# EMI-Group/evogp

Measured on AMD Instinct MI355X. Metric: tree_evals_per_s, higher is better.
Workload: dtype f32; 1 GPU; BASELINE north_star / configs[2] shape: SymbolicRegression synthetic 10-var, GLOBAL pop=1000000 x 1024 datapoints, max_tree_len=64, funcs + - * /, one tree_SR_fitness pass over every rank's shard per step; global_pop=1000000, pop_per_gpu=1000000, datapoints=1024, var_len=10, max_tree_len=64, ranks=1, device_prewarm_calls=40

## Files before the change

### evogp_amd/_lib.py

```python
from __future__ import annotations

import ctypes as C
import os

_HERE = os.path.dirname(os.path.abspath(__file__))
LIB_PATH = os.environ.get("EVOGP_HIP_LIB") or os.path.join(_HERE, "lib", "libevogp_hip.so")

ABI_VERSION = 9

_vp = C.c_void_p
_u = C.c_uint
_i = C.c_int
_f = C.c_float

PROTOTYPES = {
    "evogp_hip_generate": [_u, _u, _u, _u, _u, _f, _f, _vp, _vp, _vp, _vp, _vp, _vp, _vp, _u, _vp],
    "evogp_hip_mutate": [_i, _i, _vp, _vp, _vp, _vp, _vp, _vp, _vp, _vp, _vp, _vp, _vp],
    "evogp_hip_crossover": [_i, _i, _i, _vp, _vp, _vp, _vp, _vp, _vp, _vp, _vp, _vp, _vp, _vp],
    "evogp_hip_evaluate": [_u, _u, _u, _u, _vp, _vp, _vp, _vp, _vp, _vp],
    "evogp_hip_sr_fitness": [_u, _u, _u, _u, _u, _i, _vp, _vp, _vp, _vp, _vp, _vp, _u, _vp],
    "evogp_hip_generate_masked": [_u, _u, _u, _u, _u, _f, _f, _vp, _vp, _vp, _vp, _vp, _vp, _vp, _u, _vp, _u, _vp],
    "evogp_hip_breed_default": [_i, _i, _i, _i, _vp, _vp, _vp, _vp, _vp, _u, _vp, _vp, _vp, _vp, _vp, _vp, _vp, _vp],
    "evogp_hip_breed_default_rows": [_i, _i, _i, _i, _vp, _vp, _vp, _vp, _vp, _u, _vp, _vp, _vp, _vp, _vp, _vp, _vp, _i, _i, _vp],
    "evogp_hip_breed_default_table": [_i, _i, _i, _i, _i, _vp, _vp, _vp, _vp, _vp, _u, _vp, _vp, _vp, _vp, _vp, _vp, _vp, _i, _i, _vp],
# ... 37 lines not shown
    "evogp_hip_sr_semantic_hash_workspace_bytes": [_u, C.POINTER(C.c_ulonglong)],
    "evogp_hip_sr_semantic_hash": [_u, _u, _u, _u, _u, _vp, _vp, _vp, _vp, _vp, _vp, _vp],
    "evogp_hip_sr_semantic_classes_workspace_bytes": [_u, C.POINTER(C.c_ulonglong)],
    "evogp_hip_sr_semantic_classes": [_u, _u, _u, _u, _u, _vp, _vp, _vp, _vp, _vp, _vp, _vp, _vp],
    "evogp_hip_sr_linear_scaling": [_u, _u, _u, _u, _u, _vp, _vp, _vp, _vp, _vp, _vp, _vp, _vp],
    "evogp_hip_sr_weighted_loss": [_u, _u, _u, _u, _u, _vp, _vp, _vp, _vp, _vp, _vp, _u, _i, C.c_double, _vp, _vp],
    "evogp_hip_sr_weighted_gradient": [_u, _u, _u, _u, _u, _vp, _vp, _vp, _vp, _vp, _vp, _i, C.c_double, _vp, _vp, _vp],
    "evogp_hip_sr_weighted_normal_eq": [_u, _u, _u, _u, _u, _vp, _vp, _vp, _vp, _vp, _vp, _vp, _vp, _vp],
    "evogp_hip_sr_weighted_scaling": [_u, _u, _u, _u, _u, _vp, _vp, _vp, _vp, _vp, _vp, _u, _vp, _vp, _vp],
    "evogp_hip_sr_input_gradient": [_u, _u, _u, _u, _u, _vp, _vp, _vp, _vp, _u, _vp, _vp, _vp, _vp],
    "evogp_hip_sr_derivative_loss": [_u, _u, _u, _u, _u, _vp, _vp, _vp, _vp, _vp, _vp, _u, _vp, _vp, _vp, _vp, _vp, _vp],
    "evogp_hip_sr_gene_fitness": [_u, _u, _u, _u, _u, _vp, _vp, _vp, _vp, _vp, _vp, _vp, _vp, _vp],
    "evogp_hip_wrap_linear":[_u, _u, _u, _vp, _vp, _vp, _vp, _vp, _vp, _vp, _vp, _vp],
    "evogp_hip_tree_intervals": [_u, _u, _u, _vp, _vp, _vp, _vp, _vp, _vp, _vp, _vp, _vp],
    "evogp_hip_tree_derivative_intervals": [_u, _u, _u, _vp, _vp, _vp, _vp, _vp, _u, _vp, _vp, _vp, _vp, _vp, _vp, _vp, _vp],
    "evogp_hip_tree_dimensions": [_u, _u, _u, _u, _vp, _vp, _vp, _vp, _vp, _i, _vp, _vp, _vp, _vp],
    "evogp_hip_tree_structure": [_u, _u, _u, _vp, _vp, _vp, _vp, _vp, _vp, _vp, _vp, _i, _i, _vp, _vp, _vp, _vp, _vp, _vp, _vp],
}

DEBUG_PROTOTYPES = {
    "evogp_hip_timer_begin": [_vp],
    "evogp_hip_timer_end": [_vp, C.POINTER(C.c_float)],
    "evogp_hip_debug_set_stats": [_vp],
    "evogp_hip_debug_compile_batch": [_i],
    "evogp_hip_debug_long_compiler": [_i],
    "evogp_hip_debug_twins": [_i],
    "evogp_hip_debug_tc_fold": [_i],
    "evogp_hip_debug_tc_end": [_i],
    "evogp_hip_debug_tc_nanpeek": [_i],
    "evogp_hip_debug_tc_nanpeek_raised": [],
    "evogp_hip_debug_tc_batches": [_i, _i],
    "evogp_hip_debug_tc_table": [_i],
    "evogp_hip_debug_tc_dense": [_i],
    "evogp_hip_debug_tc_table_entry": [_i, _i, C.POINTER(C.c_uint)],
    "evogp_hip_debug_profile": [_i],
    "evogp_hip_debug_profile_read": [C.POINTER(C.c_float), C.POINTER(C.c_int)],
    "evogp_hip_debug_tc_histogram": [_u, _vp, _i, _vp],
    "evogp_hip_debug_tc_nhandlers": [],
    "evogp_hip_debug_tc_program": [_u, _vp, _i],
    "evogp_hip_debug_forget_function_classes": [],
    "evogp_hip_debug_structural_mutate_given": [_i, _i, _i, _i, _i, _vp, _vp, _vp, _vp, _vp, _vp, _vp, _vp],
    "evogp_hip_debug_insert_mutate_given": [_i, _i, _i, _vp, _vp, _vp, _vp, _vp, _vp, _vp, _vp, _vp, _vp, _vp],
    "evogp_hip_debug_point_mutate_given": [_i, _i, _i, _i, _i, _i, _i, _i, _i, _vp, _vp, _vp, _vp, _vp, _vp, _vp, _vp, _vp, _vp, _vp, _vp, _vp, _vp],
    "evogp_hip_debug_lexicase": [_vp, _i],
    "evogp_hip_debug_pareto_rank": [_i],
}


def _load() -> C.CDLL:
    if not os.path.exists(LIB_PATH):
        raise ImportError(
            f"{LIB_PATH} is missing: build the HIP engine first "
            "(python -c 'import __graft_entry__ as g; g.build()'  or  make -C evogp_amd/csrc). "
            "evogp_amd has no CPU fallback."
        )
    lib = C.CDLL(LIB_PATH)
    for name, argtypes in list(PROTOTYPES.items()) + list(DEBUG_PROTOTYPES.items()):
        fn = getattr(lib, name)
        fn.argtypes = argtypes
        fn.restype = _i
    lib.evogp_hip_evaluate_workspace_bytes.argtypes = [_u, _u]
    lib.evogp_hip_evaluate_workspace_bytes.restype = C.c_size_t
    lib.evogp_hip_select_workspace_bytes.argtypes = []
    lib.evogp_hip_select_workspace_bytes.restype = C.c_size_t
    lib.evogp_hip_program_buffer_bytes.argtypes = []
    lib.evogp_hip_program_buffer_bytes.restype = C.c_ulonglong
# ... 17 lines not shown
```

### evogp_amd/csrc/sr_tc.hip

```cpp
#include "interp.hpp"
#include "launch.hpp"
#include "sr_params.hpp"
#include "tc_interp_k8.inc"
#include "tc_interp_k4.inc"
#include "tc_interp_k1.inc"

#include <atomic>
#include <cstddef>
#include <mutex>
#include <cstdio>
#include <vector>

namespace evogp {

struct TcCompileParams {
    const float *value;
    const int16_t *type;
    const int16_t *size;
    uint2 *prog;
    float *fitness;
    unsigned *marks;
    unsigned *zero_next;
    int pop, gp_len, var_len;
    uint32_t unary_mask;
// ... 35 lines not shown
static std::atomic<int> g_fold{-1};
static std::atomic<int> g_lean_end{-1};
static std::atomic<int> g_nanpeek{-1};
static std::atomic<int> g_nanpeek_raised{0};
static std::atomic<int> g_tc_batch{0}, g_tc_dynshift{-1};
static std::atomic<int> g_compile_batch{-2};
static std::atomic<int> g_word_table{-1};
static int tc_nan_trees() {
    static const int env_fold = env_int("EVOGP_TC_FOLD", 2);
    const int fo = g_fold.load(std::memory_order_relaxed);
    return fo >= 0 ? fo : (env_fold < 0 || env_fold > 2 ? 2 : env_fold);
}
static bool tc_lean_end() {
    static const int env_end = env_int("EVOGP_TC_END", 1);
    const int le = g_lean_end.load(std::memory_order_relaxed);
    return (le >= 0 ? le : env_end) != 0;
}
static bool tc_nanpeek(long n, int num_cus) {
    static const int env_peek = env_int("EVOGP_TC_NANPEEK", 1);
    const int np = g_nanpeek.load(std::memory_order_relaxed);
    return np >= 0 ? np != 0 : (env_peek == 2 || (env_peek == 1 && n >= 900l * num_cus));
}
static bool tc_word_table() {
    static const int env_table = env_int("EVOGP_TC_TABLE", 1);
    const int wt = g_word_table.load(std::memory_order_relaxed);
    return (wt >= 0 ? wt : env_table) != 0;
}
static std::atomic<int> g_dense{-1};
static bool tc_dense() {
    static const int env_dense = env_int("EVOGP_TC_DENSE", 1);
    const int de = g_dense.load(std::memory_order_relaxed);
    return (de >= 0 ? de : env_dense) != 0;
}
static_assert(EVOGP_TC_H_LEAF_V == EVOGP_TC_H_LEAF_C + 1, "TcCompileParams::leaf_id: the variable's word is the constant's + 1, as PUSH_V is PUSH_C + 1");
static_assert(kSentinelHeavy == 0x7FC0FEEDu, "gen/gen_tc_asm.py SENTINEL_HEAVY");

__device__ inline float fold_bin4_fast(int op, float x, float y) {
    return op == 0 ? x + y : op == 1 ? x - y : op == 2 ? x * y : (y == 0.0f ? __builtin_nanf("") : x / y);
}

__device__ inline uint32_t tc_word0(int id, int slot, uint32_t pf_bytes, uint32_t aux = 0u) {
    return ((pf_bytes >> 10) << 24) | ((aux & 0xFFu) << 16) | (uint32_t)(((slot & 1) * EVOGP_TC_NHANDLERS + id) * EVOGP_TC_SLOT);
}

static_assert(EVOGP_TC_H_PUSH_V == EVOGP_TC_H_PUSH_C + 1 && EVOGP_TC_H_DIVIP_CS == EVOGP_TC_H_DIVIP_SS + 2 && EVOGP_TC_H_DIVR_CV == EVOGP_TC_H_DIVR_SV + 2 &&
              EVOGP_TC_H_PUSH_C_NP == EVOGP_TC_H_ADD_SS_NP + 24 && EVOGP_TC_H_DIVIP_SS_NP == EVOGP_TC_H_ADD_SS_NP + 26 &&
              EVOGP_TC_H_DIVR_SV_NP == EVOGP_TC_H_ADD_SS_NP + 29, "gen/gen_tc_asm.py NOPF_TWINS");
__device__ inline int no_prefetch_delta(bool arith3, bool push_c, bool in_place, bool by_recip) {
    return arith3 ? (int)EVOGP_TC_H_ADD_SS_NP : push_c ? (int)EVOGP_TC_H_PUSH_C_NP - (int)EVOGP_TC_H_PUSH_C
         : in_place ? (int)EVOGP_TC_H_DIVIP_SS_NP - (int)EVOGP_TC_H_DIVIP_SS : by_recip ? (int)EVOGP_TC_H_DIVR_SV_NP - (int)EVOGP_TC_H_DIVR_SV : 0;
}
__device__ inline bool next_word_has_variable(const TcCompileParams &, unsigned long long keptwave, bool kept, bool uses_var, bool is_root) {
    const unsigned long long U = __ballot(kept & uses_var);
    return __builtin_amdgcn_inverse_ballot_w64((((~keptwave) + (U << 1)) & keptwave) | __ballot(is_root));
}

__device__ inline void division_by_reciprocal(const TcCompileParams &p, int &id, uint32_t pf, uint32_t d1, uint32_t &aux) {
    const bool sv = id == 3 * 8 + 1, vv = id == 3 * 8 + 5, cv = id == 3 * 8 + 7;
    const bool ok = (p.recip != 0u) & (sv | vv | cv);
    const uint32_t voff = vv ? d1 << 4 : pf;
    aux = ok ? (voff + p.recip) >> 10 : aux;
    id = ok ? (int)EVOGP_TC_H_DIVR_SV + (int)vv + 2 * (int)cv : id;
}

constexpr int kUnaryInv = 10;
constexpr int kUnaryZero = 11;
// ... 1908 lines not shown
                zr = (bperm(z, rl4) & fnr) | zlr;
            }
            Mnan |= Mfn & Mop3 & B(zr != 0);
        }
    }
    const int nanincl = (int)__builtin_amdgcn_mbcnt_hi((uint32_t)(Mnan >> 32), __builtin_amdgcn_mbcnt_lo((uint32_t)Mnan, 0u)) + seli(L(Mnan), 1, 0);
    const int both = (int)((uint32_t)inclf << 15) | (nanincl << 8) | above;
    const int at_end = bperm(both, (end - 1) << 2), before = bperm(both, (lo - 1) << 2);
    const int base = seli(lo > 0, before >> 15, 0);
    const int slot = above - (at_end & 0xFF);
    const int totf = (at_end >> 15) - base;
    const int hf = seli(L(Mkept), totf - (inclf - base - deltaf), 0);
    const M Mpz = Min & B(((at_end >> 8) & 127) != seli(lo > 0, (before >> 8) & 127, 0));
    const M Mhigh = B(hf > p.depth);
    if ((Min & (~M4 | Msb | Mhigh)) != 0ull) return false;
    uint32_t ids = ent_ids;
    if (p.twins) {
        const M Uk = B((ent_bits & kTcEntUsesKept) != 0u);
        const M nxt = (((~keptwave) + (Uk << 1)) & keptwave) | Mroot;
        ids = selu(L(nxt), ids, ids >> 8);
    }
    const M Minpl = B(hf + (int)(ent_bits & kTcEntRoomMask) <= p.depth - p.div_reserve);
    const int id = (int)(selu(L(Minpl), ids >> 16, ids) & 0xFFu);
    if (L(Mkept & ~Mpz)) *(uint2 *)(rec0 + (roff + (uint32_t)slot * 8u)) = make_uint2(tc_word0(id, slot, pf, aux), d1);
    if (L(Mroot)) {
        uint32_t nan_tree = tc_word0(EVOGP_TC_H_NAN_TREE, 0, 0u);
        asm volatile("" : "+v"(nan_tree));
        const uint32_t lastw = selu(L(Mpz), nan_tree, tc_word0(p.end_id, slot + 1, p.ydelta));
        *(uint2 *)(rec0 + (roff + (uint32_t)seli(L(Mpz), 0, slot + 1) * 8u)) = make_uint2(lastw, 0u);
    }
    return true;
}

template <int B>
__global__ __launch_bounds__(256) void tc_compile_dense_kernel(TcCompileParams p) {
    typedef unsigned long long M;
    extern __shared__ uint2 tc_table_lds[];
    const int lane = threadIdx.x & 63;
    const uint32_t wave = threadIdx.x >> 6;
    const uint32_t tab = wave * (uint32_t)kTcCodes;
    {
        const int half = p.recip != 0u ? 1 : 0;
#pragma unroll
        for (int c = lane; c < kTcCodes; c += 64) {
            const uint32_t bits = kTcWordTable.bits[half][c];
            tc_table_lds[tab + (uint32_t)c] = make_uint2(kTcWordTable.ids[half][c] + ((bits & kTcEntLeaf) ? (uint32_t)p.leaf_id * 0x0101u : 0u), bits);
        }
        __builtin_amdgcn_wave_barrier();
    }
    if (p.zero_next && blockIdx.x == 0)
        for (int i = threadIdx.x; i < kCallScratchWords; i += blockDim.x) p.zero_next[i] = 0u;
    const uint32_t wave_id = uni((blockIdx.x * blockDim.x + threadIdx.x) >> 6);
    const uint32_t t0 = wave_id * (uint32_t)B;
    if (t0 >= (uint32_t)p.pop) return;
    const int nb = (int)min((uint32_t)B, (uint32_t)p.pop - t0);
    const int Lr = p.gp_len;
    uint8_t *const fnidx = (uint8_t *)(tc_table_lds + (blockDim.x >> 6) * (uint32_t)kTcCodes) + wave * (uint32_t)(B * 32);
    const size_t node0 = (size_t)t0 * (uint32_t)Lr;
    const float *const value0 = p.value + node0;
    const int16_t *const type0 = p.type + node0, *const size0 = p.size + node0;
    char *const rec0 = (char *)p.prog + (size_t)t0 * p.rec;
    int raw = 1, ty0 = T_CONST;
    float val0 = 0.0f;
    if (lane < nb) {
        const uint32_t at = (uint32_t)__mul24(lane, Lr);
        raw = (int)*(const int16_t *)((const char *)size0 + at * 2u); ty0 = (int)*(const int16_t *)((const char *)type0 + at * 2u);
        val0 = *(const float *)((const char *)value0 + at * 4u);
    }
    const int lens = lane < nb ? max(1, min(raw, Lr)) : 0;
    bool bad = __builtin_amdgcn_ballot_w64(lane < nb && (raw <= 0 || raw > Lr || (raw & 1) == 0 || (raw == 1 && ty0 != T_VAR && ty0 != T_CONST))) != 0ull;
    int nfs = 0;
    if (!bad) {
        constexpr int G = 8;
        auto load8 = [&](int (&ty)[G], int b0) {
#pragma unroll
            for (int k = 0; k < G; ++k) {
                const int len = __builtin_amdgcn_readlane(lens, (b0 + k) & 63);
                ty[k] = T_CONST;
                if (b0 + k < B && len > 1 && lane < len) ty[k] = (int)*(const int16_t *)((const char *)type0 + (uint32_t)(__mul24(b0 + k, Lr) + lane) * 2u);
            }
        };
        int cur[G], nxt[G];
        load8(cur, 0);
#pragma unroll
        for (int b0 = 0; b0 < B; b0 += G) {
            if (b0 + G < B) load8(nxt, b0 + G);
#pragma unroll
            for (int k = 0; k < G; ++k) {
                const int b = b0 + k;
                const int len = __builtin_amdgcn_readlane(lens, b);
                if (len > 1) {
                    const int ty = cur[k];
                    const M fn = __builtin_amdgcn_ballot_w64(ty == T_BFUNC);
                    const M leaf = __builtin_amdgcn_ballot_w64(ty == T_VAR) | __builtin_amdgcn_ballot_w64(ty == T_CONST);
                    const int cnt = __popcll(fn);
                    bad |= ~(fn | leaf) != 0ull || 2 * cnt + 1 != len;
                    const int rank = (int)__builtin_amdgcn_mbcnt_hi((uint32_t)(fn >> 32), __builtin_amdgcn_mbcnt_lo((uint32_t)fn, 0u));
                    if (ty == T_BFUNC && rank < 32) fnidx[b * 32 + rank] = (uint8_t)lane;
                    nfs = lane == b ? cnt : nfs;
                }
            }
#pragma unroll
            for (int k = 0; k < G; ++k) cur[k] = nxt[k];
        }
        wave_lds_sync();
    }
    bool ok = !bad;
    if (ok) {
        if (lens == 1) {
            const bool isv = ty0 == T_VAR;
            const int v = max(0, min((int)val0, p.var_len - 1));
            const uint32_t pay = isv ? (uint32_t)v * p.var_stride : f2bits(val0);
            const uint32_t id = tc_table_lds[tab + (uint32_t)(kTcCodeOther + kTcCodeRoot) + (isv ? 0u : 1u)].x & 0xFFu;
            const bool nan = !isv && p.nan_trees != 0 && (pay << 1) > 0xFF000000u;
            uint2 *const r = (uint2 *)(rec0 + (uint32_t)__mul24(lane, (int)p.rec));
            if (nan) r[0] = make_uint2(tc_word0(EVOGP_TC_H_NAN_TREE, 0, 0u), 0u);
            else {
                r[0] = make_uint2(tc_word0((int)id, 0, isv ? pay : 0u, 0u), isv ? 0u : pay);
                r[1] = make_uint2(tc_word0(p.end_id, 1, p.ydelta), 0u);
            }
        }
        int sval = nfs | (lane << 8);
#pragma unroll
        for (int r = 2; r < 5; ++r) {
            const M ones = __builtin_amdgcn_ballot_w64((sval & (1 << r)) != 0);
            const int below1 = (int)__builtin_amdgcn_mbcnt_hi((uint32_t)(ones >> 32), __builtin_amdgcn_mbcnt_lo((uint32_t)ones, 0u));
            const int to = (sval & (1 << r)) ? below1 : __popcll(ones) + lane - below1;
            sval = __builtin_amdgcn_ds_permute(to << 2, sval);
        }
        const int slen = sval & 127;
        M left = __builtin_amdgcn_ballot_w64(slen > 0);
        struct Pass { M inm; int tb, lo, nf, i, sz, tyl, szl, tyr, szr; uint32_t row; float val, vall, valr; };
        auto plan = [&](Pass &n) {
            int used = 0, about = 0;
            while (true) {
                const M cand = __builtin_amdgcn_ballot_w64(slen <= 64 - used) & left;
                if (cand == 0ull) break;
                const int j = __builtin_ctzll(cand);
                left &= ~(1ull << j);
                const int sv = __builtin_amdgcn_readlane(sval, j), l = sv & 127;
                about = (uint32_t)(lane - used) < (uint32_t)l ? (sv | (used << 16)) : about;
                used += l;
                if (used >= 64) break;
            }
            n.inm = used >= 64 ? ~0ull : (1ull << used) - 1ull;
            n.tb = (about >> 8) & 255; n.lo = about >> 16; n.nf = about & 127;
            n.row = (uint32_t)__mul24(n.tb, Lr);
            n.i = 0; n.val = (float)F_ADD; n.sz = 3; n.tyl = T_CONST; n.vall = 0.0f; n.szl = 1; n.tyr = T_CONST; n.valr = 0.0f; n.szr = 1;
            if (lane < used) {
                n.i = min((int)fnidx[n.tb * 32 + lane - n.lo], 2 * n.nf);
                const uint32_t at = n.row + (uint32_t)n.i, atl = n.row + (uint32_t)min(n.i + 1, 2 * n.nf);
                n.val = *(const float *)((const char *)value0 + at * 4u); n.sz = (int)*(const int16_t *)((const char *)size0 + at * 2u);
                n.tyl = (int)*(const int16_t *)((const char *)type0 + atl * 2u); n.vall = *(const float *)((const char *)value0 + atl * 4u);
                n.szl = (int)*(const int16_t *)((const char *)size0 + atl * 2u);
            }
        };
        auto right = [&](Pass &n) {
            if (__builtin_amdgcn_inverse_ballot_w64(n.inm)) {
                const uint32_t at = n.row + (uint32_t)dense_right_child(n.i, n.szl, n.nf);
                n.tyr = (int)*(const int16_t *)((const char *)type0 + at * 2u); n.valr = *(const float *)((const char *)value0 + at * 4u);
                n.szr = (int)*(const int16_t *)((const char *)size0 + at * 2u);
            }
        };
        Pass a = {}, b = {};
        bool have_a = left != 0ull, have_b = false;
        if (have_a) plan(a);
        have_b = left != 0ull;
        if (have_b) plan(b);
        if (have_a) right(a);
        while (have_a) {
            const Pass c = a;
            if (have_b) right(b);
            a = b; have_a = have_b;
            have_b = left != 0ull;
            if (have_b) plan(b);
            const uint32_t roff = (uint32_t)__mul24(c.tb, (int)p.rec);
            ok = compile_dense_arith(p, rec0, roff, c.inm, c.lo, c.nf, c.i, c.val, c.sz, c.tyl, c.vall, c.szl, c.tyr, c.valr, c.szr, lane, tab);
            if (!ok) break;
        }
    }
    if (!ok) tc_packed_batch<B>(p, wave_id, t0, nb, lane, tab);
}


__device__ __attribute__((always_inline)) inline int compile_long_arith(const TcCompileParams &p, char *rec0, int t, int len, char *lds, int lane,
                                                           int ty0, float val0, int sz0, int ty1, float val1, int sz1, int lds_len) {
    auto any = [](bool c) -> bool { return __builtin_amdgcn_ballot_w64(c) != 0ull; };
    auto seli = [](bool c, int x, int y) -> int { return c ? x : y; };
    auto selu = [](bool c, uint32_t x, uint32_t y) -> uint32_t { return c ? x : y; };
    const int L = lds_len;
    uint32_t *ks_s = (uint32_t *)lds;
    uint32_t *pay_s = ks_s + L;
    uint32_t *ek_s = pay_s + L;
    uint32_t *ep_s = ek_s + L;
    int32_t *offh_s = (int32_t *)(ep_s + L);
    int32_t *end_s = offh_s + L;
    int16_t *pre_s = (int16_t *)(end_s + L + 1);
    const size_t row = (size_t)t * p.gp_len;
    const int nch = (len + 63) >> 6;
    constexpr uint32_t kULo = 2u | (3u << 4) | (4u << 8) | (15u << 12) | (15u << 16) | (15u << 20) | (8u << 24) | (9u << 28);
    constexpr uint32_t kUHi = 7u | ((uint32_t)UG_INV << 4) | (15u << 8) | (0u << 12) | (1u << 16) | (5u << 20) | (6u << 24) | (15u << 28);
    for (int c = 0; c < nch; ++c) {
        const int i = c * 64 + lane;
        const bool in = i < len;
        int ty = T_CONST, sz = 1;
        float val = 0.0f;
        if (in) {
            if (c == 0) { ty = ty0; val = val0; sz = sz0; }
            else if (c == 1) { ty = ty1; val = val1; sz = sz1; }
            else { ty = (int)p.type[row + i]; val = p.value[row + i]; sz = (int)p.size[row + i]; }
        }
        const uint32_t f = (uint32_t)val;
        const bool isV = ty == T_VAR, isC = ty == T_CONST, isBf = ty == T_BFUNC, isUf = ty == T_UFUNC;
        const uint32_t fi = f - (uint32_t)F_SIN;
// ... 953 lines not shown
            for (long w = 0; w < sw && w < n; ++w) sample += (n - 1 - w) / nwaves + 1;
            *mark_sample = (int)sample;
        }
        const size_t clds = 4 * tc_general_lds_bytes(p.gp_len);
        if (clds > 64 * 1024 && !d.attr_set[15]) {
            (void)hipFuncSetAttribute((const void *)tc_compile_general_kernel<true>, hipFuncAttributeMaxDynamicSharedMemorySize, 160 * 1024 - 1024);
            (void)hipGetLastError();
            d.attr_set[15] = true;
        }
        static const int env_packed_env = env_int("EVOGP_TC_PACKED", -1);
        const int set_packed = g_compile_batch.load(std::memory_order_relaxed);
        const int env_packed = set_packed != -2 ? set_packed : env_packed_env;
        static const int env_generic = env_int("EVOGP_TC_PACK_GENERIC", 1);
        const bool packed_mo = p.out_len > 1 && env_packed != 0 && env_generic != 0;
        const bool packed = (p.out_len == 1 && env_packed != 0) || packed_mo;
        if (packed) {
            const bool un = c.nblocks != 1;
            constexpr unsigned kOwnHandlers = (1u << F_ADD) | (1u << F_SUB) | (1u << F_MUL) | (1u << F_DIV) | (1u << F_SIN) | (1u << F_COS) | (1u << F_TAN) |
                                              (1u << F_LOG) | (1u << F_LOOSE_LOG) | (1u << F_EXP) | (1u << F_INV) | (1u << F_NEG) | (1u << F_ABS) |
                                              (1u << F_SQRT) | (1u << F_LOOSE_SQRT);
            const bool may_generic = p.func_mask == 0u || (p.func_mask & ~kOwnHandlers) != 0u;
            const int mode = packed_mo ? 3 : (c.general && p.hint_general && env_generic != 0 && may_generic) ? 2 : (un || c.gp_len > 64) ? 1 : 0;
            int B = n >= 400000 ? 32 : n >= 200000 ? 16 : 8;
            if (env_packed > 0) B = env_packed >= 64 ? 64 : env_packed >= 32 ? 32 : env_packed >= 16 ? 16 : 8;
            if (mode >= 2) B = B >= 16 ? 32 : 8;
            static const int env_pwg = env_int("EVOGP_TC_PACKED_WG", 0);
            const int wgw = env_pwg == 64 ? 1 : env_pwg == 256 ? 4 : n >= 120000 ? 1 : 4;
            const long pblocks = ((long)n + wgw * B - 1) / (wgw * B);
            if (first) *mark_sample = (int)std::min<long>(n, (long)kMarkSampleBlocks * 4 * B);
            learn_packed = c.learn != 0 && mode != 3;
            nan_words = c.nan_trees >= 1 && mode != 3;
            const dim3 grid((unsigned)pblocks), wg(64 * wgw);
            const bool longrows = c.gp_len > 64;
#define EVOGP_LAUNCH_MODE(BB, MM) \
            do { if (longrows) hipLaunchKernelGGL((tc_compile_packed_kernel<BB, MM, true>), grid, wg, 0, strm, c); \
                 else hipLaunchKernelGGL((tc_compile_packed_kernel<BB, MM, false>), grid, wg, 0, strm, c); } while (0)
#define EVOGP_LAUNCH_PACKED(BB) \
            do { if (mode == 1) EVOGP_LAUNCH_MODE(BB, 1); \
                 else if (tc_word_table() && tc_dense()) hipLaunchKernelGGL((tc_compile_dense_kernel<BB>), grid, wg, (size_t)wgw * (kTcCodes * sizeof(uint2) + BB * 32), strm, c); \
                 else if (tc_word_table()) hipLaunchKernelGGL((tc_compile_packed_kernel<BB, 0, false, true>), grid, wg, (size_t)wgw * kTcCodes * sizeof(uint2), strm, c); \
                 else hipLaunchKernelGGL((tc_compile_packed_kernel<BB, 0, false>), grid, wg, 0, strm, c); } while (0)
            if (mode == 3) { if (B == 32) EVOGP_LAUNCH_MODE(32, 3); else EVOGP_LAUNCH_MODE(8, 3); }
            else if (mode == 2) { if (B == 32) EVOGP_LAUNCH_MODE(32, 2); else EVOGP_LAUNCH_MODE(8, 2); }
            else if (B == 64) EVOGP_LAUNCH_PACKED(64);
            else if (B == 32) EVOGP_LAUNCH_PACKED(32);
            else if (B == 16) EVOGP_LAUNCH_PACKED(16);
            else EVOGP_LAUNCH_PACKED(8);
#undef EVOGP_LAUNCH_PACKED
#undef EVOGP_LAUNCH_MODE
        }
        if (packed_mo) {
            hipError_t le = hipGetLastError();
            if (le != hipSuccess) return le;
            if (p.gp_len > 64) launch_marked_general(c, n, strm);
        } else if (p.out_len == 1) {
            if (!packed) hipLaunchKernelGGL(tc_compile_kernel, dim3((unsigned)cblocks), dim3(256), 0, strm, c);
            hipError_t le = hipGetLastError();
            if (le != hipSuccess) return le;
            static const bool dbg_marks = getenv("EVOGP_DEBUG_MARKS") != nullptr;
            if (dbg_marks) {
                std::vector<uint32_t> h((size_t)n);
                (void)hipStreamSynchronize(strm);
                (void)hipMemcpy(h.data(), c.fitness, (size_t)n * 4, hipMemcpyDeviceToHost);
                int shown = 0;
                for (int t = 0; t < n && shown < 4; ++t)
                    if (h[t] == kSentinelGeneral || h[t] == kSentinelHeavy) {
                        std::vector<int16_t> ty(c.gp_len), sz(c.gp_len);
                        std::vector<float> va(c.gp_len);
                        (void)hipMemcpy(ty.data(), c.type + (size_t)t * c.gp_len, c.gp_len * 2, hipMemcpyDeviceToHost);
                        (void)hipMemcpy(sz.data(), c.size + (size_t)t * c.gp_len, c.gp_len * 2, hipMemcpyDeviceToHost);
                        (void)hipMemcpy(va.data(), c.value + (size_t)t * c.gp_len, c.gp_len * 4, hipMemcpyDeviceToHost);
                        fprintf(stderr, "[evogp] tree %d left %s: len %d:", lo + t, h[t] == kSentinelGeneral ? "to the general compiler" : "marked heavy", (int)sz[0]);
// ... 360 lines not shown
            for (int i = 0; i < 32; ++i) {
                const unsigned h = (w[i].x & 0xFFFFu) / EVOGP_TC_SLOT;
                if (h >= 2u * EVOGP_TC_NHANDLERS) break;
                const unsigned id = h % EVOGP_TC_NHANDLERS;
                atomicAdd(h_s + h, 1u);
                if (id == EVOGP_TC_H_END || id == EVOGP_TC_H_END_MO || id == EVOGP_TC_H_END_CLS || id == EVOGP_TC_H_SKIP || id == EVOGP_TC_H_NAN_TREE ||
                    id == EVOGP_TC_H_END_LEAN || id == EVOGP_TC_H_LEAF_C || id == EVOGP_TC_H_LEAF_V) break;
                if (id == EVOGP_TC_H_NEXT) { r += w[i].y; more = true; break; }
            }
        }
    }
    __syncthreads();
    for (int i = threadIdx.x; i < 2 * EVOGP_TC_NHANDLERS; i += blockDim.x)
        if (h_s[i]) atomicAdd(hist + i, (unsigned long long)h_s[i]);
}

hipError_t tc_histogram(int pop, unsigned long long *hist, int hist_len, hipStream_t stream) {
    int dev = 0;
    (void)hipGetDevice(&dev);
    TcDevice &d = g_tc[dev & 63];
    std::lock_guard<std::mutex> lock(d.mu);
    if (!d.last_records || d.last_pop <= 0 || hist_len < 2 * EVOGP_TC_NHANDLERS) return hipErrorInvalidValue;
    if (pop > d.last_pop) pop = d.last_pop;
    hipError_t e = hipMemsetAsync(hist, 0, (size_t)hist_len * sizeof(unsigned long long), stream);
    if (e != hipSuccess) return e;
    hipLaunchKernelGGL(tc_histogram_kernel, dim3((unsigned)((pop + 255) / 256)), dim3(256), 0, stream, (const uint2 *)d.last_records, pop, d.last_rec, hist);
    return hipGetLastError();
}

hipError_t launch_threaded_code(const SrParams &p, hipStream_t stream, bool *handled, int *mark_sample, int *mark_chunks) {
    *handled = false;
    *mark_sample = 0;
    *mark_chunks = 1;
    if (p.results != nullptr) return hipSuccess;
    if (p.classify && p.out_len < 2) return hipSuccess;
    int k = p.D > 256 ? 8 : (p.D > 64 ? 4 : 1);
    static const int env_wide = env_int("EVOGP_TC_WIDE", 1);
    bool wide = false;
    if (p.out_len > 1 && p.out_len + 3 > EVOGP_TC_K8_DEPTH && k == 8) {
        if (env_wide && p.out_len + 3 <= EVOGP_TC_K8W_DEPTH && !p.stats) wide = true; else k = 4;
    }
    if (p.out_len > 1 && p.out_len + 3 > EVOGP_TC_K4_DEPTH && k == 4) return hipSuccess;
    if (p.out_len > 1 && p.out_len + 3 > EVOGP_TC_K1_DEPTH) return hipSuccess;
    static const int env_k = env_int("EVOGP_TC_K", 0);
    if (env_k == 1 || env_k == 4 || env_k == 8) k = env_k;
#ifndef EVOGP_FUSED_STATS
    if (p.stats) return run_tc<8, true>(p, stream, handled, mark_sample, mark_chunks);
#endif
    const int dm = sr_division_mode();
#ifdef EVOGP_FUSED_STATS
    static const int env_fused = env_int("EVOGP_TC_FUSED", 1);
#else
    static const int env_fused = env_int("EVOGP_TC_FUSED", -1);
#endif
    const bool fused_ok = k == 8 && p.out_len == 1 && !p.classify && p.gp_len <= 64 && p.marks && !p.prof_mid;
    auto fused = [&]() -> hipError_t {
        return dm == 1 ? run_fused<1>(p, stream, handled, mark_sample, mark_chunks)
             : dm == 2 ? run_fused<2>(p, stream, handled, mark_sample, mark_chunks)
                       : run_fused<0>(p, stream, handled, mark_sample, mark_chunks);
    };
    if (env_fused == 1 && fused_ok && !p.hint_general) {
        hipError_t fe = fused();
        if (fe != hipSuccess || *handled) return fe;
    }
#define EVOGP_RUN_TC(F) (wide && k == 8 ? run_tc<8, false, F, true>(p, stream, handled, mark_sample, mark_chunks) \
                        : k == 8 ? run_tc<8, false, F>(p, stream, handled, mark_sample, mark_chunks) \
// ... 23 lines not shown
}

extern "C" int evogp_hip_debug_tc_end(int mode) {
    if (mode < -1 || mode > 1) return EVOGP_E_BADARG;
    evogp::g_lean_end.store(mode, std::memory_order_relaxed);
    return EVOGP_OK;
}

extern "C" int evogp_hip_debug_tc_nanpeek(int mode) {
    if (mode < -1 || mode > 1) return EVOGP_E_BADARG;
    evogp::g_nanpeek.store(mode, std::memory_order_relaxed);
    return EVOGP_OK;
}

extern "C" int evogp_hip_debug_tc_batches(int batch, int dyn_shift) {
    if (batch < 0 || batch > 64 || dyn_shift < -1 || dyn_shift > 3) return EVOGP_E_BADARG;
    evogp::g_tc_batch.store(batch, std::memory_order_relaxed);
    evogp::g_tc_dynshift.store(dyn_shift, std::memory_order_relaxed);
    return EVOGP_OK;
}

extern "C" int evogp_hip_debug_tc_nanpeek_raised(void) { return evogp::g_nanpeek_raised.load(std::memory_order_relaxed); }

extern "C" int evogp_hip_debug_tc_table(int mode) {
    if (mode < -1 || mode > 1) return EVOGP_E_BADARG;
    evogp::g_word_table.store(mode, std::memory_order_relaxed);
    return EVOGP_OK;
}

extern "C" int evogp_hip_debug_tc_dense(int mode) {
    if (mode < -1 || mode > 1) return EVOGP_E_BADARG;
    evogp::g_dense.store(mode, std::memory_order_relaxed);
    return EVOGP_OK;
}

extern "C" int evogp_hip_debug_tc_table_entry(int recip, int code, unsigned *entry) {
    if (recip < 0 || recip > 1 || code < 0 || code >= evogp::kTcCodes || !entry) return EVOGP_E_BADARG;
    entry[0] = evogp::kTcWordTableHost.ids[recip][code];
    entry[1] = evogp::kTcWordTableHost.bits[recip][code];
    return EVOGP_OK;
}

extern "C" int evogp_hip_debug_long_compiler(int fast) {
    if (fast < -1 || fast > 1) return EVOGP_E_BADARG;
    evogp::g_long_fast.store(fast, std::memory_order_relaxed);
    return EVOGP_OK;
}

extern "C" int evogp_hip_debug_compile_batch(int trees) {
    if (trees < -1 || trees > 64) return EVOGP_E_BADARG;
    evogp::g_compile_batch.store(trees, std::memory_order_relaxed);
    return EVOGP_OK;
}

extern "C" int evogp_hip_set_program_buffer_limit(unsigned long long bytes) {
    evogp::g_prog_limit.store(bytes, std::memory_order_relaxed);
    return EVOGP_OK;
}

extern "C" int evogp_hip_set_allocator(evogp_alloc_fn alloc, evogp_free_fn free_fn) {
    if ((alloc == nullptr) != (free_fn == nullptr)) return EVOGP_E_BADARG;
    for (auto &d : evogp::g_tc) {
        std::lock_guard<std::mutex> lock(d.mu);
        if (d.prog || d.graph_prog || !d.retired.empty() || !d.rings.empty() || d.spare_ring) return EVOGP_E_BADARG;
    }
    if (evogp::grad_workspaces_held() || evogp::case_workspaces_held()) return EVOGP_E_BADARG;
// ... 87 lines not shown
```

### include/evogp_hip_debug.h

```cpp
#ifndef EVOGP_HIP_DEBUG_H
#define EVOGP_HIP_DEBUG_H
#include "evogp_hip.h"
#ifdef __cplusplus
extern "C" {
#endif

int evogp_hip_timer_begin(evogp_stream_t stream);
int evogp_hip_timer_end(evogp_stream_t stream, float *elapsed_ms);

int evogp_hip_debug_set_stats(unsigned long long *device_counters);

int evogp_hip_debug_profile(int enable);
int evogp_hip_debug_profile_read(float *stage_ms , int *calls);

int evogp_hip_debug_compile_batch(int trees);
int evogp_hip_debug_long_compiler(int fast);
int evogp_hip_debug_twins(int mode);
int evogp_hip_debug_tc_fold(int mode);
int evogp_hip_debug_tc_end(int mode);
int evogp_hip_debug_tc_nanpeek(int mode);
int evogp_hip_debug_tc_nanpeek_raised(void);
int evogp_hip_debug_tc_batches(int batch, int dyn_shift);
int evogp_hip_debug_tc_table(int mode);
int evogp_hip_debug_tc_dense(int mode);
int evogp_hip_debug_tc_table_entry(int recip, int code, unsigned *entry);

int evogp_hip_debug_tc_histogram(unsigned pop, unsigned long long *device_hist, int hist_len, evogp_stream_t stream);
int evogp_hip_debug_tc_nhandlers(void);
int evogp_hip_debug_tc_program(unsigned tree, unsigned *host_words, int max_words);

int evogp_hip_debug_forget_function_classes(void);

int evogp_hip_debug_structural_mutate_given(int pop_size, int gp_len, int mode, int inner_is_offset, int skip_rows, const int *given,
                                            const float *value, const int16_t *type, const int16_t *size, float *value_res,
                                            int16_t *type_res, int16_t *size_res, evogp_stream_t stream);
int evogp_hip_debug_insert_mutate_given(int pop_size, int gp_len, int skip_rows, const int *given, const float *value, const int16_t *type,
                                        const int16_t *size, const float *donor_value, const int16_t *donor_type, const int16_t *donor_size,
                                        float *value_res, int16_t *type_res, int16_t *size_res, evogp_stream_t stream);
int evogp_hip_debug_point_mutate_given(int pop_size, int gp_len, int mode, int modify_output, int fix_roulette, int skip_rows, int input_len,
                                       int output_len, int n_consts, const unsigned char *target, const float *u, const int *var_idx,
                                       const int *const_idx, const int *out_idx, const float *value, const int16_t *type, const int16_t *size,
                                       const float *roulette_ufuncs, const float *roulette_bfuncs, const float *roulette_tfuncs,
                                       const float *const_samples, float *value_res, evogp_stream_t stream);

int evogp_hip_debug_lexicase(unsigned long long *device_counters, int stop_after);

int evogp_hip_debug_pareto_rank(int stop_after);

#ifdef __cplusplus
}
#endif
#endif
```

Baseline: 1930 billion tree-evals/s.

## Restructure dense tree compiler node stage with packed per-node metadata in LDS

The dense compile kernel's node scan now has each lane read four nodes at once with 8-byte loads. It covers four trees per wave step, classifies nodes with packed 16-bit ops, ranks function nodes with a DPP prefix scan, and writes a per-node meta byte (size and type class) to LDS. The plan stage then reads child sizes and types from that LDS meta instead of reloading type and size from global memory, and drops the separate right-child prefetch pass. It also loads child values only for leaves. The dense path is now taken only when gp_len is a multiple of four and the type and size buffers are 8-byte aligned. A device counter of fallbacks to the packed compiler is added for debugging, at the cost of more LDS per wave.

```diff
diff --git a/evogp_amd/_lib.py b/evogp_amd/_lib.py
--- a/evogp_amd/_lib.py
+++ b/evogp_amd/_lib.py
@@ -93,6 +93,7 @@
     "evogp_hip_debug_tc_batches": [_i, _i],
     "evogp_hip_debug_tc_table": [_i],
     "evogp_hip_debug_tc_dense": [_i],
+    "evogp_hip_debug_tc_dense_fallbacks": [],
     "evogp_hip_debug_tc_table_entry": [_i, _i, C.POINTER(C.c_uint)],
     "evogp_hip_debug_profile": [_i],
     "evogp_hip_debug_profile_read": [C.POINTER(C.c_float), C.POINTER(C.c_int)],
diff --git a/evogp_amd/csrc/sr_tc.hip b/evogp_amd/csrc/sr_tc.hip
--- a/evogp_amd/csrc/sr_tc.hip
+++ b/evogp_amd/csrc/sr_tc.hip
@@ -91,6 +91,7 @@
     const int de = g_dense.load(std::memory_order_relaxed);
     return (de >= 0 ? de : env_dense) != 0;
 }
+static std::atomic<unsigned *> g_dense_fallbacks{nullptr};
 static_assert(EVOGP_TC_H_LEAF_V == EVOGP_TC_H_LEAF_C + 1, "TcCompileParams::leaf_id: the variable's word is the constant's + 1, as PUSH_V is PUSH_C + 1");
 static_assert(kSentinelHeavy == 0x7FC0FEEDu, "gen/gen_tc_asm.py SENTINEL_HEAVY");
 
@@ -2065,6 +2066,7 @@
     return true;
 }
 
+constexpr int kMarkDenseFallbacks = 16;
 template <int B>
 __global__ __launch_bounds__(256) void tc_compile_dense_kernel(TcCompileParams p) {
     typedef unsigned long long M;
@@ -2088,7 +2090,8 @@
     if (t0 >= (uint32_t)p.pop) return;
     const int nb = (int)min((uint32_t)B, (uint32_t)p.pop - t0);
     const int Lr = p.gp_len;
-    uint8_t *const fnidx = (uint8_t *)(tc_table_lds + (blockDim.x >> 6) * (uint32_t)kTcCodes) + wave * (uint32_t)(B * 32);
+    uint8_t *const fnidx = (uint8_t *)(tc_table_lds + (blockDim.x >> 6) * (uint32_t)kTcCodes) + wave * (uint32_t)(B * 96);
+    uint8_t *const meta = fnidx + B * 32;
     const size_t node0 = (size_t)t0 * (uint32_t)Lr;
     const float *const value0 = p.value + node0;
     const int16_t *const type0 = p.type + node0, *const size0 = p.size + node0;
@@ -2104,38 +2107,78 @@
     bool bad = __builtin_amdgcn_ballot_w64(lane < nb && (raw <= 0 || raw > Lr || (raw & 1) == 0 || (raw == 1 && ty0 != T_VAR && ty0 != T_CONST))) != 0ull;
     int nfs = 0;
     if (!bad) {
-        constexpr int G = 8;
-        auto load8 = [&](int (&ty)[G], int b0) {
+        static_assert(B % 4 == 0 && T_VAR == 0 && T_CONST == 1 && T_BFUNC == 3, "the node stage's groups of four trees and its meta byte");
+        constexpr int NG = B / 4, G = 2;
+        const int q = lane >> 4, j4 = (lane & 15) << 2;
+        struct Quad { uint2 ty, sz; int len; };
+        auto load = [&](Quad &c, int g) {
+            const int l = __builtin_amdgcn_ds_bpermute((4 * g + q) << 2, lens);
+            c.len = l > 1 ? l : 0;
+            c.ty = make_uint2(0x00010001u, 0x00010001u);
+            c.sz = c.ty;
+            if (j4 < c.len) {
+                const uint32_t at = (uint32_t)(__mul24(4 * g + q, Lr) + j4) * 2u;
+                c.ty = *(const uint2 *)((const char *)type0 + at); c.sz = *(const uint2 *)((const char *)size0 + at);
+            }
+        };
+        constexpr uint32_t kOnes = 0x00010001u;
+        auto pk_min = [](uint32_t x, uint32_t c) -> uint32_t { uint32_t r; asm("v_pk_min_u16 %0, %1, %2" : "=v"(r) : "v"(x), "s"(c)); return r; };
+        auto pk_add = [](uint32_t x, uint32_t c) -> uint32_t { uint32_t r; asm("v_pk_add_u16 %0, %1, %2" : "=v"(r) : "v"(x), "s"(c)); return r; };
+        auto pk_shr1 = [](uint32_t x) -> uint32_t { uint32_t r; asm("v_pk_lshrrev_b16 %0, 1, %1 op_sel_hi:[0,1]" : "=v"(r) : "v"(x)); return r; };
+        uint32_t odd = 0u;
+        auto stage = [&](const Quad &c, int g) {
+            const int nlive = c.len - j4;
+            const uint32_t live[2] = {nlive >= 2 ? ~0u : 0xFFFFu, nlive >= 4 ? ~0u : nlive >= 2 ? 0xFFFFu : 0u};
+            const uint32_t tw[2] = {c.ty.x, c.ty.y}, sw[2] = {c.sz.x, c.sz.y};
+            uint32_t fn[2], half[2];
 #pragma unroll
-            for (int k = 0; k < G; ++k) {
-                const int len = __builtin_amdgcn_readlane(lens, (b0 + k) & 63);
-                ty[k] = T_CONST;
-                if (b0 + k < B && len > 1 && lane < len) ty[k] = (int)*(const int16_t *)((const char *)type0 + (uint32_t)(__mul24(b0 + k, Lr) + lane) * 2u);
-            }
+            for (int d = 0; d < 2; ++d) {
+                uint32_t t = (tw[d] & live[d]) | (kOnes & ~live[d]);
+                asm("" : "+v"(t));
+                const uint32_t s1 = pk_add((sw[d] & live[d]) | (kOnes & ~live[d]), 0xFFFFFFFFu);
+                const uint32_t cls = pk_min(t, 2u * kOnes);
+                const uint32_t other = pk_min(t ^ ((uint32_t)T_BFUNC * kOnes), kOnes);
+                fn[d] = other ^ kOnes;
+                odd |= pk_shr1(cls) & other;
+                odd |= s1 & 0xFFC0FFC0u;
+                half[d] = (s1 & 0x003F003Fu) | (cls << 6);
+            }
+            const uint32_t both = fn[0] + fn[1];
+            const int cnt = (int)((both & 0xFFFFu) + (both >> 16));
+            int incl = cnt;
+            incl += __builtin_amdgcn_update_dpp(0, incl, kDppRowShr | 1, 0xf, 0xf, true);
+            incl += __builtin_amdgcn_update_dpp(0, incl, kDppRowShr | 2, 0xf, 0xf, true);
+            incl += __builtin_amdgcn_update_dpp(0, incl, kDppRowShr | 4, 0xf, 0xf, true);
+            incl += __builtin_amdgcn_update_dpp(0, incl, kDppRowShr | 8, 0xf, 0xf, true);
+            asm("" : "+v"(incl));
+            uint8_t *const fi = fnidx + (4 * g + q) * 32;
+            const int is[4] = {(int)(fn[0] & 1u), (int)(fn[0] >> 16), (int)(fn[1] & 1u), (int)(fn[1] >> 16)};
+            int rank = incl - cnt;
+#pragma unroll
+            for (int k = 0; k < 4; ++k) {
+                asm("" : "+v"(rank));
+                if (is[k]) fi[rank] = (uint8_t)(j4 + k);
+                rank += is[k];
+            }
+            *(uint32_t *)(meta + (4 * g + q) * 64 + j4) = __builtin_amdgcn_perm(half[1], half[0], 0x06040200u);
+            const int got = __builtin_amdgcn_ds_bpermute((((lane & 3) << 4) + 15) << 2, incl);
+            nfs = (lane >> 2) == g ? got : nfs;
         };
-        int cur[G], nxt[G];
-        load8(cur, 0);
+        Quad cur[G], nxt[G] = {};
 #pragma unroll
-        for (int b0 = 0; b0 < B; b0 += G) {
-            if (b0 + G < B) load8(nxt, b0 + G);
+        for (int k = 0; k < G; ++k) load(cur[k], k);
+#pragma unroll 1
+        for (int g0 = 0; g0 < NG; g0 += G) {
+            if (g0 + G < NG) {
 #pragma unroll
-            for (int k = 0; k < G; ++k) {
-                const int b = b0 + k;
-                const int len = __builtin_amdgcn_readlane(lens, b);
-                if (len > 1) {
-                    const int ty = cur[k];
-                    const M fn = __builtin_amdgcn_ballot_w64(ty == T_BFUNC);
-                    const M leaf = __builtin_amdgcn_ballot_w64(ty == T_VAR) | __builtin_amdgcn_ballot_w64(ty == T_CONST);
-                    const int cnt = __popcll(fn);
-                    bad |= ~(fn | leaf) != 0ull || 2 * cnt + 1 != len;
-                    const int rank = (int)__builtin_amdgcn_mbcnt_hi((uint32_t)(fn >> 32), __builtin_amdgcn_mbcnt_lo((uint32_t)fn, 0u));
-                    if (ty == T_BFUNC && rank < 32) fnidx[b * 32 + rank] = (uint8_t)lane;
-                    nfs = lane == b ? cnt : nfs;
-                }
-            }
+                for (int k = 0; k < G; ++k) load(nxt[k], g0 + G + k);
+            }
+#pragma unroll
+            for (int k = 0; k < G; ++k) stage(cur[k], g0 + k);
 #pragma unroll
             for (int k = 0; k < G; ++k) cur[k] = nxt[k];
         }
+        bad |= __builtin_amdgcn_ballot_w64(odd != 0u || (lens > 1 && 2 * nfs + 1 != lens)) != 0ull;
         wave_lds_sync();
     }
     bool ok = !bad;
@@ -2163,7 +2206,7 @@
         }
         const int slen = sval & 127;
         M left = __builtin_amdgcn_ballot_w64(slen > 0);
-        struct Pass { M inm; int tb, lo, nf, i, sz, tyl, szl, tyr, szr; uint32_t row; float val, vall, valr; };
+        struct Pass { M inm; int tb, lo, nf, i, sz, tyl, szl, tyr, szr; float val, vall, valr; };
         auto plan = [&](Pass &n) {
             int used = 0, about = 0;
             while (true) {
@@ -2178,41 +2221,39 @@
             }
             n.inm = used >= 64 ? ~0ull : (1ull << used) - 1ull;
             n.tb = (about >> 8) & 255; n.lo = about >> 16; n.nf = about & 127;
-            n.row = (uint32_t)__mul24(n.tb, Lr);
             n.i = 0; n.val = (float)F_ADD; n.sz = 3; n.tyl = T_CONST; n.vall = 0.0f; n.szl = 1; n.tyr = T_CONST; n.valr = 0.0f; n.szr = 1;
             if (lane < used) {
+                const uint8_t *const m = meta + n.tb * 64;
                 n.i = min((int)fnidx[n.tb * 32 + lane - n.lo], 2 * n.nf);
-                const uint32_t at = n.row + (uint32_t)n.i, atl = n.row + (uint32_t)min(n.i + 1, 2 * n.nf);
-                n.val = *(const float *)((const char *)value0 + at * 4u); n.sz = (int)*(const int16_t *)((const char *)size0 + at * 2u);
-                n.tyl = (int)*(const int16_t *)((const char *)type0 + atl * 2u); n.vall = *(const float *)((const char *)value0 + atl * 4u);
-                n.szl = (int)*(const int16_t *)((const char *)size0 + atl * 2u);
+                const int li = min(n.i + 1, 2 * n.nf);
+                const uint32_t mi = m[n.i], ml = m[li];
+                n.sz = (int)(mi & 63u) + 1; n.szl = (int)(ml & 63u) + 1;
+                const int ri = dense_right_child(n.i, n.szl, n.nf);
+                const uint32_t mr = m[ri];
+                n.szr = (int)(mr & 63u) + 1;
+                n.tyl = (int)((ml >> 6) + (ml >> 7)); n.tyr = (int)((mr >> 6) + (mr >> 7));
+                const uint32_t row = (uint32_t)__mul24(n.tb, Lr);
+                n.val = *(const float *)((const char *)value0 + (row + (uint32_t)n.i) * 4u);
+                if (n.tyl != T_BFUNC) n.vall = *(const float *)((const char *)value0 + (row + (uint32_t)li) * 4u);
+                if (n.tyr != T_BFUNC) n.valr = *(const float *)((const char *)value0 + (row + (uint32_t)ri) * 4u);
             }
         };
-        auto right = [&](Pass &n) {
-            if (__builtin_amdgcn_inverse_ballot_w64(n.inm)) {
-                const uint32_t at = n.row + (uint32_t)dense_right_child(n.i, n.szl, n.nf);
-                n.tyr = (int)*(const int16_t *)((const char *)type0 + at * 2u); n.valr = *(const float *)((const char *)value0 + at * 4u);
-                n.szr = (int)*(const int16_t *)((const char *)size0 + at * 2u);
-            }
-        };
-        Pass a = {}, b = {};
-        bool have_a = left != 0ull, have_b = false;
-        if (have_a) plan(a);
-        have_b = left != 0ull;
-        if (have_b) plan(b);
-        if (have_a) right(a);
-        while (have_a) {
+        Pass a = {};
+        bool have = left != 0ull;
+        if (have) plan(a);
+        while (have) {
             const Pass c = a;
-            if (have_b) right(b);
-            a = b; have_a = have_b;
-            have_b = left != 0ull;
-            if (have_b) plan(b);
+            have = left != 0ull;
+            if (have) plan(a);
             const uint32_t roff = (uint32_t)__mul24(c.tb, (int)p.rec);
             ok = compile_dense_arith(p, rec0, roff, c.inm, c.lo, c.nf, c.i, c.val, c.sz, c.tyl, c.vall, c.szl, c.tyr, c.valr, c.szr, lane, tab);
             if (!ok) break;
         }
     }
-    if (!ok) tc_packed_batch<B>(p, wave_id, t0, nb, lane, tab);
+    if (!ok) {
+        if (lane == 0 && p.marks) atomicAdd(p.marks + kMarkDenseFallbacks, 1u);
+        tc_packed_batch<B>(p, wave_id, t0, nb, lane, tab);
+    }
 }
 
 
@@ -3232,12 +3273,15 @@
             nan_words = c.nan_trees >= 1 && mode != 3;
             const dim3 grid((unsigned)pblocks), wg(64 * wgw);
             const bool longrows = c.gp_len > 64;
+            const bool dense = mode == 0 && !longrows && tc_word_table() && tc_dense() && c.gp_len % 4 == 0 &&
+                               (((uintptr_t)c.type | (uintptr_t)c.size) & 7u) == 0u;
+            g_dense_fallbacks.store(dense && c.marks ? c.marks + kMarkDenseFallbacks : nullptr, std::memory_order_relaxed);
 #define EVOGP_LAUNCH_MODE(BB, MM) \
             do { if (longrows) hipLaunchKernelGGL((tc_compile_packed_kernel<BB, MM, true>), grid, wg, 0, strm, c); \
                  else hipLaunchKernelGGL((tc_compile_packed_kernel<BB, MM, false>), grid, wg, 0, strm, c); } while (0)
 #define EVOGP_LAUNCH_PACKED(BB) \
             do { if (mode == 1) EVOGP_LAUNCH_MODE(BB, 1); \
-                 else if (tc_word_table() && tc_dense()) hipLaunchKernelGGL((tc_compile_dense_kernel<BB>), grid, wg, (size_t)wgw * (kTcCodes * sizeof(uint2) + BB * 32), strm, c); \
+                 else if (dense) hipLaunchKernelGGL((tc_compile_dense_kernel<BB>), grid, wg, (size_t)wgw * (kTcCodes * sizeof(uint2) + BB * 96), strm, c); \
                  else if (tc_word_table()) hipLaunchKernelGGL((tc_compile_packed_kernel<BB, 0, false, true>), grid, wg, (size_t)wgw * kTcCodes * sizeof(uint2), strm, c); \
                  else hipLaunchKernelGGL((tc_compile_packed_kernel<BB, 0, false>), grid, wg, 0, strm, c); } while (0)
             if (mode == 3) { if (B == 32) EVOGP_LAUNCH_MODE(32, 3); else EVOGP_LAUNCH_MODE(8, 3); }
@@ -3664,6 +3708,7 @@
     *handled = false;
     *mark_sample = 0;
     *mark_chunks = 1;
+    g_dense_fallbacks.store(nullptr, std::memory_order_relaxed);
     if (p.results != nullptr) return hipSuccess;
     if (p.classify && p.out_len < 2) return hipSuccess;
     int k = p.D > 256 ? 8 : (p.D > 64 ? 4 : 1);
@@ -3753,6 +3798,13 @@
     if (mode < -1 || mode > 1) return EVOGP_E_BADARG;
     evogp::g_dense.store(mode, std::memory_order_relaxed);
     return EVOGP_OK;
+}
+
+extern "C" int evogp_hip_debug_tc_dense_fallbacks(void) {
+    const unsigned *const word = evogp::g_dense_fallbacks.load(std::memory_order_relaxed);
+    unsigned n = 0u;
+    if (!word || hipDeviceSynchronize() != hipSuccess || hipMemcpy(&n, word, sizeof n, hipMemcpyDeviceToHost) != hipSuccess) return -1;
+    return (int)n;
 }
 
 extern "C" int evogp_hip_debug_tc_table_entry(int recip, int code, unsigned *entry) {
diff --git a/include/evogp_hip_debug.h b/include/evogp_hip_debug.h
--- a/include/evogp_hip_debug.h
+++ b/include/evogp_hip_debug.h
@@ -23,6 +23,7 @@
 int evogp_hip_debug_tc_batches(int batch, int dyn_shift);
 int evogp_hip_debug_tc_table(int mode);
 int evogp_hip_debug_tc_dense(int mode);
+int evogp_hip_debug_tc_dense_fallbacks(void);
 int evogp_hip_debug_tc_table_entry(int recip, int code, unsigned *entry);
 
 int evogp_hip_debug_tc_histogram(unsigned pop, unsigned long long *device_hist, int hist_len, evogp_stream_t stream);
```

Result: faster. 1996 billion tree-evals/s (median of 6 runs) (+3.4%).
